# daultanigaurav/AI-BASED-FRAME-INTERPOLATION

Measured on AMD Instinct MI355X. Metric: interpolated frames/sec at 1080p, higher is better.
Workload: dtype bf16

## Files before the change

### ai_based_frame_interpolation_amd/_native.py

```python
from __future__ import annotations

import ctypes
import os
import subprocess

import torch

_PKG = os.path.dirname(os.path.abspath(__file__))
LIB_PATH = os.environ.get("FIUNET_LIB") or os.path.join(_PKG, "libfiunet_hip.so")
CSRC = os.path.join(_PKG, "csrc")

ABI_VERSION = 8
ABI_MIN_COMPAT = 4
FP32, BF16, BF16X2, FP16 = 0, 1, 2, 3
OPT_UNFUSED, OPT_KEEP_ALL, OPT_GATHER_UPSAMPLE = 1, 2, 16
OPT_RNE_WEIGHTS, OPT_NO_DITHER = 32, 64
WEIGHT_PREPS = ("host", "device")
YUV_MPEG2, YUV_BT709, YUV_FULL_RANGE, YUV_BT2020 = 1, 2, 4, 8

SYMBOLS = (
    "fiunet_abi_version", "fiunet_last_error_string", "fiunet_create", "fiunet_destroy",
    "fiunet_set_options", "fiunet_load_weights", "fiunet_load_weights_device", "fiunet_prepare_precision", "fiunet_workspace_bytes", "fiunet_forward",
    "fiunet_min_unsplit_batch",
    "fiunet_forward_strip",
    "fiunet_workspace_bytes_u8", "fiunet_forward_u8", "fiunet_forward_u8_strided", "fiunet_preprocess_u8",
    "fiunet_postprocess_u8", "fiunet_debug_read_activation", "fiunet_profile_enable",
    "fiunet_profile_read", "fiunet_metrics_workspace_bytes", "fiunet_psnr_u8", "fiunet_ssim_u8",
    "fiunet_ssim_gauss_workspace_bytes", "fiunet_ssim_gauss_f32",
    "fiunet_plane_metrics_workspace_bytes", "fiunet_plane_psnr", "fiunet_plane_ssim",
    "fiunet_yuv420_to_rgb_u8", "fiunet_rgb_to_yuv420_u8", "fiunet_workspace_bytes_yuv420", "fiunet_forward_yuv420",
    "fiunet_preprocess_p10", "fiunet_postprocess_p10", "fiunet_workspace_bytes_p10", "fiunet_forward_p10",
    "fiunet_yuv420p10_to_rgb_p10", "fiunet_rgb_p10_to_yuv420p10", "fiunet_workspace_bytes_yuv420p10",
    "fiunet_forward_yuv420p10",
    "fiunet_pair_sad_u8", "fiunet_pair_sad_p10", "fiunet_scene_cuts", "fiunet_hold_cut_frames",
    "fiunet_retime_u8", "fiunet_retime_p10",
    "fiunet_yuv_to_rgb_u8", "fiunet_rgb_to_yuv_u8", "fiunet_yuv_to_rgb_p10", "fiunet_rgb_p10_to_yuv",
    "fiunet_workspace_bytes_yuv", "fiunet_forward_yuv", "fiunet_forward_yuv_p10",
    "fiunet_packed_to_rgb_u8", "fiunet_rgb_to_packed_u8", "fiunet_workspace_bytes_rgb_packed",
    "fiunet_forward_rgb_packed",
    "fiunet_nv12_to_rgb_u8", "fiunet_rgb_to_nv12_u8", "fiunet_workspace_bytes_nv12", "fiunet_forward_nv12",
    "fiunet_p010_to_rgb_p10", "fiunet_rgb_p10_to_p010", "fiunet_workspace_bytes_p010", "fiunet_forward_p010",
)


class SurfaceLayout(ctypes.Structure):
    _fields_ = [("luma_pitch", ctypes.c_size_t), ("chroma_offset", ctypes.c_size_t),
                ("chroma_pitch", ctypes.c_size_t), ("frame_stride", ctypes.c_size_t)]


def _surface(layout, frame_stride: int):
    if layout is None:
        return ctypes.byref(SurfaceLayout(0, 0, 0, frame_stride))
    return ctypes.byref(SurfaceLayout(layout.luma_pitch, layout.chroma_offset, layout.chroma_pitch, frame_stride))



class PackedLayout(ctypes.Structure):
    _fields_ = [("row_pitch", ctypes.c_size_t), ("frame_stride", ctypes.c_size_t)]


def _packed(layout, frame_stride: int):
    return ctypes.byref(PackedLayout(layout.row_pitch, frame_stride))

_lib = None


def build(force: bool = False) -> str:
    if force and os.path.exists(LIB_PATH):
        os.remove(LIB_PATH)
# ... 486 lines not shown
```

### ai_based_frame_interpolation_amd/csrc/conv3x3_mfma.hip.h

```cpp
#pragma once
#include <hip/hip_runtime.h>
#include <stdint.h>
#include <type_traits>

namespace fiunet {

typedef __attribute__((ext_vector_type(4))) float f32x4;
typedef __attribute__((ext_vector_type(8))) __bf16 bf16x8;
typedef __attribute__((ext_vector_type(8))) _Float16 f16x8;

enum SrcMode { SRC_DIRECT = 0, SRC_POOL = 1 , SRC_CONCAT_UP = 2,
               SRC_STEM = 3 ,
               SRC_DIRECT_X2 = 4,
               SRC_STEM_X2 = 5 };
constexpr bool src_is_stem(int mode) { return mode == SRC_STEM || mode == SRC_STEM_X2; }
constexpr bool src_is_x2(int mode) { return mode == SRC_DIRECT_X2 || mode == SRC_STEM_X2; }

__device__ __forceinline__ size_t blk_off(int plane, int y, int x, int H, int W)
{
    return (((size_t)plane * H + y) * W + x) * 64;
}

struct ConvArgs {
    const void* src0;
    const void* src1;
    const void* wgt;
    const float* scale;
    const float* shift;
    void* dst;
    void* pool_dst;
    int B, H, W;
    int C0, C1, Cout;
    int lowH, lowW;
    int padT, padL;
    float sy, sx;
    int upOffY;
    int lowOffY;
    int lowHg;
    int tilesX, tilesY, nct;
    int relu;
    const float* f1;
    const float* f2;
    const void* stem_w;
    float dither;
    int ksplit;
    float* kslab;
    unsigned long long* stamp;
    unsigned stamp_cap;
    const float* head_w;
    const float* head_b;
    float* head_out;
    const uint8_t* u1;
    const uint8_t* u2;
    uint8_t* head_out_u8;
    int head_nc;
    size_t head_img_stride;
};

template <typename T> struct Elem;
template <> struct Elem<float> {
    static constexpr int PL = 16;
    static constexpr int NE = 4;
};
template <> struct Elem<__bf16> {
    static constexpr int PL = 32;
    static constexpr int NE = 8;
};
template <> struct Elem<_Float16> {
    static constexpr int PL = 32;
    static constexpr int NE = 8;
};

template <typename T> __device__ __forceinline__ void chunk_unpack(const uint4& c, float* f);
template <> __device__ __forceinline__ void chunk_unpack<float>(const uint4& c, float* f)
{
    f[0] = __uint_as_float(c.x); f[1] = __uint_as_float(c.y);
    f[2] = __uint_as_float(c.z); f[3] = __uint_as_float(c.w);
}
template <> __device__ __forceinline__ void chunk_unpack<__bf16>(const uint4& c, float* f)
{
    f[0] = __uint_as_float(c.x << 16); f[1] = __uint_as_float(c.x & 0xffff0000u);
    f[2] = __uint_as_float(c.y << 16); f[3] = __uint_as_float(c.y & 0xffff0000u);
    f[4] = __uint_as_float(c.z << 16); f[5] = __uint_as_float(c.z & 0xffff0000u);
    f[6] = __uint_as_float(c.w << 16); f[7] = __uint_as_float(c.w & 0xffff0000u);
}
template <> __device__ __forceinline__ void chunk_unpack<_Float16>(const uint4& c, float* f)
{
    typedef __attribute__((ext_vector_type(2))) _Float16 f16x2;
    const f16x2 a = __builtin_bit_cast(f16x2, c.x), b = __builtin_bit_cast(f16x2, c.y);
    const f16x2 d = __builtin_bit_cast(f16x2, c.z), e = __builtin_bit_cast(f16x2, c.w);
    f[0] = (float)a[0]; f[1] = (float)a[1]; f[2] = (float)b[0]; f[3] = (float)b[1];
    f[4] = (float)d[0]; f[5] = (float)d[1]; f[6] = (float)e[0]; f[7] = (float)e[1];
}
// ... 309 lines not shown
    static constexpr int LDS_BYTES = STEMW_OFF + STEMW_BYTES;
    static_assert(LDS_BYTES <= 80 * 1024, "two workgroups must fit in the CU's 160 KiB of LDS");
    static_assert(!src_is_stem(MODE) || LDS_BYTES <= 63 * 1280, "fused-stem kernel: stay below 64 LDS granules");
};

constexpr int conv_wave_frags(int BN, int TH, int TW) { return TH * TW / 16 / (4 / (BN / 64)); }
constexpr int conv_occupancy(int BN, int TH, int TW, int lds_bytes = 0)
{
    return conv_wave_frags(BN, TH, TW) == 4 && lds_bytes * 3 <= 160 * 1024 ? 3 : 2;
}


__device__ __forceinline__ int conv_block_remap()
{
    const int nblk = gridDim.x, bid = blockIdx.x;
    const int q = nblk >> 3, r = nblk & 7, xcd = bid & 7;
    return (xcd < r ? xcd * (q + 1) : r * (q + 1) + (xcd - r) * q) + (bid >> 3);
}

struct ConvTileId { int ct, b, ty, tx; };
__device__ __forceinline__ ConvTileId conv_tile_decode(const ConvArgs& a, int t)
{
    ConvTileId d;
    d.ct = t % a.nct; t /= a.nct;
    d.tx = t % a.tilesX; t /= a.tilesX;
    d.ty = t % a.tilesY;
    d.b = t / a.tilesY;
    return d;
}

template <typename T> __device__ __forceinline__ int conv_cout_ofs(int m, int lc)
{
    return sizeof(T) == 2 ? (m >> 1) * 32 + lc * 8 + (m & 1) * 4 : m * 16 + lc * 4;
}

template <typename T, int BN, int TH, int TW, int EPI>
__device__ __forceinline__ void conv_acc_init(const ConvArgs& a, f32x4 (&acc)[4][conv_wave_frags(BN, TH, TW)],
                                              int ct, int wc, int lc)
{
    constexpr int NF = conv_wave_frags(BN, TH, TW);
#pragma unroll
    for (int m = 0; m < 4; ++m) {
        f32x4 v = f32x4{0.f, 0.f, 0.f, 0.f};
        if constexpr (!epi_is_splitk(EPI)) {
            const float4 sh = *reinterpret_cast<const float4*>(a.shift + ct * BN + wc * 64 + conv_cout_ofs<T>(m, lc));
            v = f32x4{sh.x, sh.y, sh.z, sh.w};
        }
#pragma unroll
        for (int n = 0; n < NF; ++n) acc[m][n] = v;
    }
}

__device__ __forceinline__ unsigned relu_pk_bf16(unsigned p) { return pk_max_i16(p, 0u); }
__device__ __forceinline__ void relu_fma(float& sum, float x, float lo, float w)
{
    float t;
    asm("v_max_f32 %1, %3, %2\n\tv_fmac_f32 %0, %1, %4" : "+v"(sum), "=&v"(t) : "v"(x), "v"(lo), "v"(w));
}

template <typename T, int BN, int TH, int TW, int EPI, bool X2 = false>
__device__ __forceinline__ void conv_epilogue(const ConvArgs& a, f32x4 (&acc)[4][conv_wave_frags(BN, TH, TW)],
                                              int b, int y0, int x0, int ct, int split, int wc, int wp,
                                              int l15, int lc)
{
    constexpr int PL = Elem<T>::PL;
    constexpr int FR = TW / 16;
    constexpr int NF = conv_wave_frags(BN, TH, TW);
    constexpr int ROWS_W = NF / FR;
    constexpr int HNC = EPI == EPI_HEAD ? 1 : (EPI == EPI_HEAD3 ? 3 : 0);
    const int aH = a.H, aW = a.W;
    constexpr bool PERM = sizeof(T) == 2;
    const int wbase_c = ct * BN + wc * 64;
    if constexpr (epi_is_splitk(EPI)) {
        const int tile = (((b * a.tilesY) + y0 / TH) * a.tilesX + x0 / TW) * a.nct + ct;
        const int ntile = a.B * a.tilesY * a.tilesX * a.nct;
        const int wave = wp * (BN / 64) + wc;
        float4* o = reinterpret_cast<float4*>(a.kslab) + ((((size_t)split * ntile + tile) * 4 + wave) * (4 * NF)) * 64 + (lc * 16 + l15);
#pragma unroll
        for (int m = 0; m < 4; ++m)
#pragma unroll
            for (int n = 0; n < NF; ++n)
                o[(m * NF + n) * 64] = make_float4(acc[m][n][0], acc[m][n][1], acc[m][n][2], acc[m][n][3]);
        return;
    }
    float hw[HNC > 0 ? HNC : 1][4][4];
#pragma unroll
    for (int c = 0; c < HNC; ++c)
#pragma unroll
        for (int m = 0; m < 4; ++m) {
            const float4 v = *reinterpret_cast<const float4*>(a.head_w + c * 64 + conv_cout_ofs<T>(m, lc));
            hw[c][m][0] = v.x; hw[c][m][1] = v.y; hw[c][m][2] = v.z; hw[c][m][3] = v.w;
        }
    const size_t plane_stride = (size_t)aH * aW * 64;
    const int plane0 = wbase_c / PL;
    const int rec_byte = lc * 16;
    char* const out_img = a.dst ? (char*)a.dst + (size_t)b * plane_stride * (a.Cout / PL) +
                                  (size_t)plane0 * plane_stride + rec_byte : nullptr;
    const int pH = aH >> 1, pW = aW >> 1;
    const size_t pplane_stride = (size_t)pH * pW * 64;
    char* const pool_img = EPI == EPI_POOL ? (char*)a.pool_dst + (size_t)b * pplane_stride * (a.Cout / PL) +
                                             (size_t)plane0 * pplane_stride + rec_byte : nullptr;
    if constexpr (HNC > 0) {
        static_assert(HNC == 0 || NF == 8 || NF == 4, "head reduction is written for 8 or 4 fragments per wave");
        const float floor_v = a.relu ? 0.f : -__builtin_inff();
        float hb[HNC];
#pragma unroll
        for (int c = 0; c < HNC; ++c) hb[c] = a.head_b[c];
        const int nb = ((lc & 1) ? 4 : 0) + ((lc & 2) ? 2 : 0);
#pragma unroll
        for (int c = 0; c < HNC; ++c) {
            float hs[NF];
#pragma unroll
            for (int n = 0; n < NF; ++n) {
                float sum = 0.f;
#pragma unroll
                for (int m = 0; m < 4; ++m)
#pragma unroll
                    for (int j = 0; j < 4; ++j) relu_fma(sum, acc[m][n][j], floor_v, hw[c][m][j]);
                hs[n] = sum;
            }
            if constexpr (NF == 4) {
                float full[NF];
#pragma unroll
                for (int n = 0; n < NF; ++n) {
                    const float p = hs[n] + __shfl_xor(hs[n], 16);
                    full[n] = p + __shfl_xor(p, 32);
                }
                const float mine = lc == 0 ? full[0] : (lc == 1 ? full[1] : (lc == 2 ? full[2] : full[3]));
                const int n = lc;
                const int y = y0 + wp * ROWS_W + n / FR;
                const int x = x0 + (n % FR) * 16 + l15;
                if (y < aH && x < aW) {
                    const size_t o = (size_t)b * a.head_img_stride + ((size_t)c * aH + y) * aW + x;
                    if (a.head_out_u8) a.head_out_u8[o] = postprocess_u8_value(mine + hb[c]);
                    else a.head_out[o] = mine + hb[c];
                }
            } else {
                float t[4], u[2];
#pragma unroll
                for (int i = 0; i < 4; ++i) {
                    const auto r = __builtin_amdgcn_permlane16_swap(__float_as_uint(hs[i]), __float_as_uint(hs[(i + 4) % NF]), false, false);
                    t[i] = __uint_as_float(r[0]) + __uint_as_float(r[1]);
                }
#pragma unroll
                for (int j = 0; j < 2; ++j) {
                    const auto r = __builtin_amdgcn_permlane32_swap(__float_as_uint(t[j]), __float_as_uint(t[j + 2]), false, false);
                    u[j] = __uint_as_float(r[0]) + __uint_as_float(r[1]);
                }
#pragma unroll
                for (int j = 0; j < 2; ++j) {
                    const int n = nb + j;
                    const int y = y0 + wp * ROWS_W + n / FR;
                    const int x = x0 + (n % FR) * 16 + l15;
                    if (y < aH && x < aW) {
                        const size_t o = (size_t)b * a.head_img_stride + ((size_t)c * aH + y) * aW + x;
                        if (a.head_out_u8) a.head_out_u8[o] = postprocess_u8_value(u[j] + hb[c]);
                        else a.head_out[o] = u[j] + hb[c];
                    }
                }
            }
        }
    }
    if constexpr (X2) {
        static_assert(std::is_same_v<T, __bf16>, "the two-piece epilogue belongs to the bf16 kernels");
        if (HNC > 0 && !a.dst) return;
        const size_t ps = (size_t)aH * aW * 64;
        const int npo = a.Cout / 32;
        const size_t blk = (size_t)npo * ps;
        char* const img = (char*)a.dst + (size_t)b * 2 * blk + (size_t)(wbase_c / 32) * ps + lc * 16;
        const int pH2 = aH >> 1, pW2 = aW >> 1;
        const size_t pps = (size_t)pH2 * pW2 * 64, pblk = (size_t)npo * pps;
        char* const pimg = EPI == EPI_POOL ? (char*)a.pool_dst + (size_t)b * 2 * pblk + (size_t)(wbase_c / 32) * pps + lc * 16
                                           : nullptr;
        auto put = [&](char* o, size_t block_bytes, const float (&v)[8]) __attribute__((always_inline)) {
            unsigned h[4], l[4];
#pragma unroll
            for (int i = 0; i < 4; ++i) {
                h[i] = pack_bf16x2_pk(v[2 * i], v[2 * i + 1]);
                l[i] = pack_bf16x2_pk(v[2 * i] - __uint_as_float(h[i] << 16), v[2 * i + 1] - __uint_as_float(h[i] & 0xffff0000u));
            }
            *reinterpret_cast<uint4*>(o) = make_uint4(h[0], h[1], h[2], h[3]);
            *reinterpret_cast<uint4*>(o + block_bytes) = make_uint4(l[0], l[1], l[2], l[3]);
        };
#pragma unroll
        for (int n = 0; n < NF; ++n) {
            const int y = y0 + wp * ROWS_W + n / FR;
            const int x = x0 + (n % FR) * 16 + l15;
            if (y < aH && x < aW) {
#pragma unroll
                for (int g = 0; g < 2; ++g) {
                    float v[8];
#pragma unroll
                    for (int j = 0; j < 4; ++j) {
                        v[j] = a.relu ? fmaxf(acc[2 * g][n][j], 0.f) : acc[2 * g][n][j];
                        v[4 + j] = a.relu ? fmaxf(acc[2 * g + 1][n][j], 0.f) : acc[2 * g + 1][n][j];
                    }
                    put(img + (size_t)(y * aW + x) * 64 + g * ps, blk, v);
                }
            }
        }
        if constexpr (EPI == EPI_POOL) {
#pragma unroll
            for (int n = 0; n < NF; ++n) {
                if (((n / FR) & 1) != 0) continue;
                const int y = y0 + wp * ROWS_W + n / FR;
                const int x = x0 + (n % FR) * 16 + l15;
                const int py = y >> 1, px = x >> 1;
                const bool okp = (py < pH2) && (px < pW2) && ((l15 & 1) == 0);
#pragma unroll
                for (int g = 0; g < 2; ++g) {
                    float v[8];
#pragma unroll
                    for (int h = 0; h < 2; ++h)
// ... 10 lines not shown
        }
        return;
    }
    if constexpr (EPI == EPI_POOL && PERM) {
#pragma unroll
        for (int n = 0; n < NF; ++n) {
            if (((n / FR) & 1) != 0) continue;
            uint4 pk[2][2];
#pragma unroll
            for (int r = 0; r < 2; ++r) {
                const int nn = n + r * FR;
                const int y = y0 + wp * ROWS_W + nn / FR;
                const int x = x0 + (nn % FR) * 16 + l15;
                const bool ok = (y < aH) && (x < aW);
                char* o = out_img + (size_t)(y * aW + x) * 64;
#pragma unroll
                for (int g = 0; g < 2; ++g) {
                    uint4 v = make_uint4(pack2_pk<T>(acc[2 * g][nn][0], acc[2 * g][nn][1]),
                                         pack2_pk<T>(acc[2 * g][nn][2], acc[2 * g][nn][3]),
                                         pack2_pk<T>(acc[2 * g + 1][nn][0], acc[2 * g + 1][nn][1]),
                                         pack2_pk<T>(acc[2 * g + 1][nn][2], acc[2 * g + 1][nn][3]));
                    if (a.relu) v = make_uint4(relu_pk_bf16(v.x), relu_pk_bf16(v.y), relu_pk_bf16(v.z), relu_pk_bf16(v.w));
                    pk[r][g] = v;
                    if (ok && out_img) *reinterpret_cast<uint4*>(o + g * plane_stride) = v;
                }
            }
            const int y = y0 + wp * ROWS_W + n / FR;
            const int x = x0 + (n % FR) * 16 + l15;
            const int py = y >> 1, px = x >> 1;
            const bool okp = (py < pH) && (px < pW) && ((l15 & 1) == 0);
            char* o = pool_img + (size_t)(min(py, pH - 1) * pW + min(px, pW - 1)) * 64;
#pragma unroll
            for (int g = 0; g < 2; ++g) {
                const uint4 t = pk[0][g], u = pk[1][g];
                const unsigned c0 = pk_max_i16(t.x, u.x), c1 = pk_max_i16(t.y, u.y);
                const unsigned c2 = pk_max_i16(t.z, u.z), c3 = pk_max_i16(t.w, u.w);
                const uint4 m = make_uint4(pk_max_i16(c0, dpp_swap_pairs(c0)), pk_max_i16(c1, dpp_swap_pairs(c1)),
                                           pk_max_i16(c2, dpp_swap_pairs(c2)), pk_max_i16(c3, dpp_swap_pairs(c3)));
                if (okp) *reinterpret_cast<uint4*>(o + g * pplane_stride) = m;
            }
        }
        return;
    }
#pragma unroll
    for (int n = 0; n < NF; ++n) {
        const int y = y0 + wp * ROWS_W + n / FR;
        const int x = x0 + (n % FR) * 16 + l15;
        const bool ok = (y < aH) && (x < aW);
        if (ok && out_img) {
            char* o = out_img + (size_t)(y * aW + x) * 64;
            if constexpr (PERM) {
#pragma unroll
                for (int g = 0; g < 2; ++g) {
                    uint4 pk = make_uint4(pack2<T>(acc[2 * g][n][0], acc[2 * g][n][1]),
                                          pack2<T>(acc[2 * g][n][2], acc[2 * g][n][3]),
                                          pack2<T>(acc[2 * g + 1][n][0], acc[2 * g + 1][n][1]),
                                          pack2<T>(acc[2 * g + 1][n][2], acc[2 * g + 1][n][3]));
                    if (a.relu) pk = make_uint4(relu_pk_bf16(pk.x), relu_pk_bf16(pk.y), relu_pk_bf16(pk.z), relu_pk_bf16(pk.w));
                    *reinterpret_cast<uint4*>(o + g * plane_stride) = pk;
                }
            } else {
#pragma unroll
                for (int m = 0; m < 4; ++m) {
                    float4 v = make_float4(acc[m][n][0], acc[m][n][1], acc[m][n][2], acc[m][n][3]);
                    if (a.relu) v = make_float4(fmaxf(v.x, 0.f), fmaxf(v.y, 0.f), fmaxf(v.z, 0.f), fmaxf(v.w, 0.f));
                    *reinterpret_cast<float4*>(o + m * plane_stride) = v;
                }
            }
        }
    }
    if (EPI == EPI_POOL) {
#pragma unroll
        for (int n = 0; n < NF; ++n) {
            if (((n / FR) & 1) != 0) continue;
            const int y = y0 + wp * ROWS_W + n / FR;
            const int x = x0 + (n % FR) * 16 + l15;
            const int py = y >> 1, px = x >> 1;
            const bool okp = (py < pH) && (px < pW) && ((l15 & 1) == 0);
            char* o = pool_img + (size_t)(min(py, pH - 1) * pW + min(px, pW - 1)) * 64;
            if constexpr (!PERM) {
#pragma unroll
                for (int m = 0; m < 4; ++m) {
                    float r[4];
#pragma unroll
                    for (int j = 0; j < 4; ++j) {
                        const float cm = fmaxf(acc[m][n][j], acc[m][n + FR][j]);
                        r[j] = fmaxf(cm, __uint_as_float(dpp_swap_pairs(__float_as_uint(cm))));
                        if (a.relu) r[j] = fmaxf(r[j], 0.f);
                    }
                    if (okp) *reinterpret_cast<float4*>(o + m * pplane_stride) = make_float4(r[0], r[1], r[2], r[3]);
                }
            } else {
#pragma unroll
                for (int g = 0; g < 2; ++g) {
                    unsigned r[4];
#pragma unroll
                    for (int h = 0; h < 2; ++h) {
                        const int m = 2 * g + h;
                        const unsigned a0 = pk_max_i16(pack2_pk<T>(acc[m][n][0], acc[m][n][1]),
                                                       pack2_pk<T>(acc[m][n + FR][0], acc[m][n + FR][1]));
                        const unsigned a1 = pk_max_i16(pack2_pk<T>(acc[m][n][2], acc[m][n][3]),
                                                       pack2_pk<T>(acc[m][n + FR][2], acc[m][n + FR][3]));
                        r[2 * h] = pk_max_i16(a0, dpp_swap_pairs(a0));
                        r[2 * h + 1] = pk_max_i16(a1, dpp_swap_pairs(a1));
                        if (a.relu) { r[2 * h] = relu_pk_bf16(r[2 * h]); r[2 * h + 1] = relu_pk_bf16(r[2 * h + 1]); }
                    }
                    if (okp) *reinterpret_cast<uint4*>(o + g * pplane_stride) = make_uint4(r[0], r[1], r[2], r[3]);
                }
            }
        }
// ... 545 lines not shown
                }
            } else {
#pragma unroll
                for (int ky = 0; ky < 3; ++ky) {
                    asm volatile("" ::: "memory");
                    uint4 wa[4], xb[NF];
#pragma unroll
                    for (int m = 0; m < 4; ++m)
                        wa[m] = *reinterpret_cast<const uint4*>(wcur + (ky * BN + m * 16) * 64);
#pragma unroll
                    for (int n = 0; n < NF; ++n)
                        xb[n] = *reinterpret_cast<const uint4*>(
                            lds_in + b_off[kx] + (((n / FR) + ky) * TWP + (n % FR) * 16) * 64);
#pragma unroll
                    for (int m = 0; m < 4; ++m)
#pragma unroll
                        for (int n = 0; n < NF; ++n) mma_chunk<T>(acc[m][n], wa[m], xb[n]);
                }
            }
#ifdef FIUNET_STAMP
            asm volatile("" :: "v"(acc[3][NF - 1][3]));
            __builtin_amdgcn_sched_barrier(0);
#endif
            STAMP(2);
            if (kx == 2 && gather_next && !early) {
                __syncthreads();
                gather_plane(plane + 1, step & 1, false);
                lds_dma_wait_all();
                __syncthreads();
                if constexpr (STEM && X2) { if (plane + 1 == 2) stem_park(1); }
                STAMP(4);
            } else {
                lds_dma_wait_all();
                __syncthreads();
                STAMP(3);
            }
        }
    }

#ifdef FIUNET_CLOCK
    {
        asm volatile("" :: "v"(acc[3][NF - 1][3]));
        __builtin_amdgcn_sched_barrier(0);
        const unsigned long long ck_t1 = __builtin_amdgcn_s_memtime(), ck_r1 = __builtin_amdgcn_s_memrealtime();
        const unsigned st_idx = blockIdx.x * 4u + (unsigned)wave;
        if (a.stamp && lane == 0 && st_idx < a.stamp_cap) {
            unsigned long long* rec = a.stamp + (size_t)st_idx * 16;
            rec[0] = ck_t1 - ck_t0;
            rec[1] = ck_r1 - ck_r0;
            rec[8] = 1ull;
        }
    }
#endif
    conv_epilogue<T, BN, TH, TW, EPI, X2>(a, acc, b, y0, x0, ct, split, wc, wp, l15, lc);
#ifdef FIUNET_STAMP
    STAMP(5);
    st_sum[0] = st_prev - st_t0;
    const unsigned st_idx = blockIdx.x * 4u + (unsigned)wave;
    if (a.stamp && lane == 0 && st_idx < a.stamp_cap) {
        unsigned long long* rec = a.stamp + (size_t)st_idx * 16;
#pragma unroll
        for (int k = 0; k < 16; ++k) rec[k] = k == 8 ? 1ull : st_sum[k];
    }
#endif
}

template <typename T, int BN, int TH, int TW, int EPI, bool X2>
__global__ __launch_bounds__(64) void splitk_finalize_tile_kernel(const ConvArgs a)
{
    static_assert(EPI == EPI_PLAIN || EPI == EPI_POOL, "a fused head is never K-split");
    constexpr int WAVES_C = BN / 64;
    constexpr int NF = conv_wave_frags(BN, TH, TW);
    int t = blockIdx.x >> 2;
    const int tile = t;
    const int ct = t % a.nct; t /= a.nct;
    const int tx = t % a.tilesX; t /= a.tilesX;
    const int ty = t % a.tilesY;
    const int b = t / a.tilesY;
    const int lane = threadIdx.x & 63, wave = blockIdx.x & 3;
    const int l15 = lane & 15, lc = lane >> 4;
    const int wc = wave % WAVES_C, wp = wave / WAVES_C;
    const int ntile = a.B * a.tilesY * a.tilesX * a.nct;
    f32x4 acc[4][NF];
#pragma unroll
    for (int m = 0; m < 4; ++m)
#pragma unroll
        for (int n = 0; n < NF; ++n) acc[m][n] = f32x4{0.f, 0.f, 0.f, 0.f};
    const float4* p = reinterpret_cast<const float4*>(a.kslab) + (((size_t)tile * 4 + wave) * (4 * NF)) * 64 + lane;
    const size_t slice = (size_t)ntile * 4 * (4 * NF) * 64;
    const int ks = a.ksplit;
#pragma unroll
    for (int m = 0; m < 4; ++m) {
        const float4* pm = p + (size_t)m * NF * 64;
        constexpr int CH = NF == 8 ? 2 : 4;
        for (int s0 = 0; s0 < ks; s0 += CH, pm += CH * slice) {
            float4 q[CH][NF];
#pragma unroll
            for (int j = 0; j < CH; ++j)
                if (s0 + j < ks) {
#pragma unroll
                    for (int n = 0; n < NF; ++n) q[j][n] = pm[j * slice + n * 64];
                }
#pragma unroll
            for (int j = 0; j < CH; ++j)
                if (s0 + j < ks) {
#pragma unroll
                    for (int n = 0; n < NF; ++n) {
// ... 18 lines not shown
```

### ai_based_frame_interpolation_amd/csrc/fiunet.hip

```cpp
#include "../../include/fiunet.h"
#include "pointwise.hip.h"
#include "conv3x3_kwave.hip.h"
#include "metrics.hip.h"
#include "colour.hip.h"
#include "packed.hip.h"
#include "yuv4xx.hip.h"
#include "scene.hip.h"
#include "retime.hip.h"
#include "weights.hip.h"

#include <algorithm>
#include <atomic>
#include <cmath>
#include <cstdio>
#include <cstring>
#include <map>
#include <string>
#include <vector>

using namespace fiunet;

namespace {

thread_local std::string g_err;
// ... 539 lines not shown
        HIP_TRY(hipEventRecord(ev[0], s));
    }
    const float dither = bf16 && !(ctx->flags & FIUNET_OPT_NO_DITHER) ? 0.00390625f : 0.f;
    const ConvWeights& c0 = ctx->conv[0];
    const double stem_flops = 2.0 * B * H * W * 9.0 * c0.cin * c0.cout;
    if (L[0].form == STEM_RGB_SPLIT) {
        const long long ntiles = (long long)B * ((H + 15) / 16) * ((W + 31) / 32);
        const dim3 g2((unsigned)std::min<long long>(ntiles, 256 * FIUNET_RGB_STEM_OCC));
        if (x2)
            hipLaunchKernelGGL(stem_rgb_split_kernel<true>, g2, dim3(256), 0, s, f1, f2, (const float*)c0.w_f32, c0.scale,
                               c0.shift, (__bf16*)act(0), B, H, W, dither, u1, u2);
        else if (f16)
            hipLaunchKernelGGL((stem_rgb_split_kernel<false, _Float16>), g2, dim3(256), 0, s, f1, f2, (const float*)c0.w_f32, c0.scale,
                               c0.shift, (_Float16*)act(0), B, H, W, 0.f, u1, u2);
        else
            hipLaunchKernelGGL(stem_rgb_split_kernel<false>, g2, dim3(256), 0, s, f1, f2, (const float*)c0.w_f32, c0.scale,
                               c0.shift, (__bf16*)act(0), B, H, W, dither, u1, u2);
        HIP_TRY(hipGetLastError());
    } else if (L[0].form == STEM_FIRST) {
        const long long nruns = (long long)B * H * (((W + 15) / 16 + 7) / 8);
        const dim3 grid((unsigned)std::min<long long>((nruns + 3) / 4, 256 * 64));
        if (x2)
            hipLaunchKernelGGL((conv3x3_first_kernel<__bf16, 1, true>), grid, dim3(256), 0, s, f1, f2, (const float*)c0.w_f32,
                               c0.scale, c0.shift, (__bf16*)act(0), B, H, W, dither);
        else if (ctx->cf == 1)
            hipLaunchKernelGGL((conv3x3_first_kernel<T, 1>), grid, dim3(256), 0, s, f1, f2, (const float*)c0.w_f32, c0.scale,
                               c0.shift, (T*)act(0), B, H, W, dither);
        else if constexpr (sizeof(T) == 4)
            hipLaunchKernelGGL((conv3x3_first_kernel<T, 3>), grid, dim3(256), 0, s, f1, f2, (const float*)c0.w_f32, c0.scale,
                               c0.shift, (T*)act(0), B, H, W, dither);
        HIP_TRY(hipGetLastError());
    }
    if (ev) {
        HIP_TRY(hipEventRecord(ev[1], s));
        if (L[0].form == STEM_FUSED) ctx->layer_name[0] = "(stem fused into next stage)";
        else if (x2) ctx->layer_name[0] = L[0].form == STEM_FIRST ? "conv3x3_first_kernel<f32 arithmetic, two-piece output>"
                                                                  : "stem_rgb_split_kernel<two-piece output>";
        else ctx->layer_name[0] = L[0].form == STEM_FIRST ? std::string("conv3x3_first_kernel<") + elem_name<T>() + "," +
                                                                std::to_string(ctx->cf) + ">"
                                                          : std::string(f16 ? "stem_rgb_split_kernel<fp16 output>" : "stem_rgb_split_kernel");
        ctx->layer_flops[0] = L[0].form == STEM_FUSED ? 0.0 : stem_flops;
    }
    for (int i = 1; i < NCONV; ++i) {
        const StageLaunch& st = L[i];
        const ConvWeights& cw = ctx->conv[i];
        const int lv = kLevel[i];
        ConvArgs a;
        std::memset(&a, 0, sizeof(a));
        a.B = B; a.H = p.hs[lv]; a.W = p.ws[lv];
        a.Cout = cw.cout;
        a.wgt = x2 ? cw.w_x2 : bf16 ? cw.w_bf16 : f16 ? cw.w_f16 : cw.w_f32;
        a.scale = cw.scale; a.shift = cw.shift;
        a.relu = 1;
        a.ksplit = 1;
        a.kslab = st.slab ? (float*)(ws + p.slab_off) : nullptr;
        a.stamp = (ctx->stamps && i == ctx->stamp_layer) ? ctx->stamps : nullptr;
        a.stamp_cap = (unsigned)kStampWaves;
        a.dst = st.stored ? act(i) : nullptr;
        a.src0 = act(kSrc0[i]);
        a.C0 = ctx->cout[kSrc0[i]];
        int mode = x2 ? SRC_DIRECT_X2 : SRC_DIRECT;
        if (st.form == FORM_POOL) {
            char* pooled = ws + p.pool_off[lv - 1];
            if (L[i - 1].epi != EPI_POOL) {
                const size_t n = (size_t)B * a.H * a.W * (a.C0 * sizeof(T) / 16);
                hipLaunchKernelGGL((maxpool2_kernel<T>), dim3(grid_for(n)), dim3(256), 0, s,
                                   (const T*)a.src0, (T*)pooled, B, p.hs[lv - 1], p.ws[lv - 1], a.C0);
                HIP_TRY(hipGetLastError());
            }
            a.src0 = pooled;
        } else if (kMode[i] == SRC_CONCAT_UP) {
            a.src1 = act(kSrc1[i]);
            a.C1 = ctx->cout[kSrc1[i]];
            a.lowH = p.hs[lv + 1]; a.lowW = p.ws[lv + 1];
            a.lowHg = hg[lv + 1];
            a.upOffY = y_origin >> lv;
            a.lowOffY = y_origin >> (lv + 1);
            const int dy = hg[lv] - 2 * a.lowHg, dx = a.W - 2 * a.lowW;
            a.padT = dy / 2; a.padL = dx / 2;
            a.sy = 2 * a.lowHg > 1 ? (float)(a.lowHg - 1) / (float)(2 * a.lowHg - 1) : 0.f;
            a.sx = 2 * a.lowW > 1 ? (float)(a.lowW - 1) / (float)(2 * a.lowW - 1) : 0.f;
            char* up = ws + p.up_off[i];
            if (st.form == FORM_CONCAT_CONVT) {
                const auto& ct = ctx->convt[(i - 10) / 2];
                ConvTArgs c;
                std::memset(&c, 0, sizeof(c));
                c.low = a.src1; c.wgt = x2 ? ct.w_x2 : bf16 ? ct.w_bf16 : f16 ? ct.w_f16 : ct.w_f32; c.bias = ct.bias; c.dst = up;
                c.B = B; c.H = a.H; c.W = a.W; c.lowH = a.lowH; c.lowW = a.lowW; c.Cin = ct.cin; c.Cout = ct.cout;
                c.padT = a.padT; c.padL = a.padL; c.upOffY = a.upOffY; c.lowOffY = a.lowOffY; c.lowHg = a.lowHg;
                if (a.C1 != ct.cin) return fail(FIUNET_ERR_INVALID_ARG, "internal: transposed-conv channel plan mismatch");
                if (y_origin != 0 || Hg != H || a.H != 2 * a.lowH || a.W != 2 * a.lowW)
                    HIP_TRY(hipMemsetAsync(up, 0, (size_t)B * a.H * a.W * ct.cout * es, s));
                const long long units = (long long)B * a.lowH * ((a.lowW + 31) / 32) * (ct.cout / 64);
                const dim3 grid((unsigned)std::min<long long>((units + 3) / 4, 256 * 16));
                if (x2) {
                    if constexpr (std::is_same_v<T, __bf16>) hipLaunchKernelGGL((convt2x2_kernel<T, true>), grid, dim3(256), 0, s, c);
                } else
                    hipLaunchKernelGGL((convt2x2_kernel<T>), grid, dim3(256), 0, s, c);
                HIP_TRY(hipGetLastError());
                a.src1 = up; a.C1 = ct.cout;
            } else if (st.form == FORM_CONCAT_UPCAT) {
                T* scratch = (T*)(ws + p.scratch_off);
                const size_t n = (size_t)B * a.H * a.W * ((a.C0 + a.C1) * sizeof(T) / 16);
                hipLaunchKernelGGL((upcat_kernel<T>), dim3(grid_for(n)), dim3(256), 0, s, a, scratch);
                HIP_TRY(hipGetLastError());
                a.src0 = scratch; a.C0 = a.C0 + a.C1; a.C1 = 0; a.src1 = nullptr;
// ... 1531 lines not shown
    return retime(grid, n_intervals, frame_samples, depth, first_interval, j0, n_out, p, q, mode, flags, out, stream);
}

int fiunet_retime_p10(const uint16_t* grid, int n_intervals, size_t frame_samples, int depth, uint64_t first_interval,
                      uint64_t j0, int n_out, uint32_t p, uint32_t q, int mode, const uint8_t* flags, uint16_t* out,
                      void* stream)
{
    return retime(grid, n_intervals, frame_samples, depth, first_interval, j0, n_out, p, q, mode, flags, out, stream);
}

int fiunet_debug_force_cfg(fiunet_ctx* ctx, int layer, int tile, int ksplit)
{
    if (!ctx || layer >= NCONV || tile < 0 || tile > 3 || ksplit < 0 || ksplit > 32)
        return fail(FIUNET_ERR_INVALID_ARG, "fiunet_debug_force_cfg: bad arguments");
    if (layer < 0) {
        for (int i = 0; i < NCONV; ++i) ctx->force_tile[i] = ctx->force_ksplit[i] = 0;
        return FIUNET_OK;
    }
    ctx->force_tile[layer] = tile;
    ctx->force_ksplit[layer] = ksplit;
    return FIUNET_OK;
}

int fiunet_debug_weight_buffer(const fiunet_ctx* ctx, int layer, int which, const void** ptr, size_t* bytes)
{
    if (!ctx || !ptr || !bytes || layer < 0 || layer > NCONV + 4 || which < 0 || which > 5)
        return fail(FIUNET_ERR_INVALID_ARG, "fiunet_debug_weight_buffer: bad arguments");
    if (!ctx->loaded) return fail(FIUNET_ERR_NOT_LOADED, "fiunet_debug_weight_buffer before a load");
    const void* p = nullptr;
    size_t b = 0;
    if (layer < NCONV) {
        const ConvWeights& cw = ctx->conv[layer];
        const size_t nel = (size_t)9 * cw.cin * cw.cout;
        if (which == 0) { p = cw.scale; b = (size_t)cw.cout * 4; }
        else if (which == 1) { p = cw.shift; b = (size_t)cw.cout * 4; }
        else if (which == 2) { p = cw.w_f32; b = nel * 4; }
        else if (which == 3) { p = cw.w_bf16; b = nel * 2; }
        else if (which == 4 && layer == 0) { p = ctx->stem_w_split; b = (size_t)2 * 64 * 32 * 2; }
    } else if (layer < NCONV + 4) {
        const auto& ct = ctx->convt[layer - NCONV];
        const size_t nel = (size_t)4 * ct.cin * ct.cout;
        if (which == 2) { p = ct.w_f32; b = nel * 4; }
        else if (which == 3) { p = ct.w_bf16; b = nel * 2; }
        else if (which == 5) { p = ct.bias; b = (size_t)ct.cout * 4; }
    } else {
        if (which == 2) { p = ctx->head_w; b = (size_t)ctx->cf * 64 * 4; }
        else if (which == 5) { p = ctx->head_b; b = (size_t)ctx->cf * 4; }
    }
    *ptr = p;
    *bytes = p ? b : 0;
    return FIUNET_OK;
}

int fiunet_debug_choose_cfg(int precision, int B, int H, int W, int Cin, int Cout, int splittable, int concat_stage,
                            int kwave_ok, int* out )
{
    if (!out || B < 1 || H < 1 || W < 1 || Cin < 32 || (Cout != 64 && Cout % 128 != 0) || !valid_precision(precision))
        return fail(FIUNET_ERR_INVALID_ARG, "fiunet_debug_choose_cfg: bad arguments");
    const bool concat = concat_stage >= 10;
    out[3] = concat && concat_stage < NCONV && kMode[concat_stage] == SRC_CONCAT_UP &&
             (precision == FIUNET_BF16X2 ||
              materialise_up(precision, B, H, W, conv_cin(kCoutBil, true, concat_stage), kCoutBil[concat_stage]));
    const ConvCfg c = choose_conv_cfg(precision == FIUNET_FP32, precision == FIUNET_BF16X2, B, H, W, Cin, Cout, splittable != 0,
                                      -1, 0, concat ? out[3] != 0 : kwave_ok != 0, kwave_ok != 0,
                                      concat && !(precision == FIUNET_FP32 && out[3]));
    out[0] = c.small; out[1] = c.ksplit; out[2] = c.kwave;
    return FIUNET_OK;
}

int fiunet_debug_stage_cfg(int frame_channels, int bilinear, unsigned flags, int precision, int B, int H, int W, int stage,
                           int* out )
{
    if (!out || (frame_channels != 1 && frame_channels != 3) || B < 1 || H < 16 || W < 16 || stage < 0 || stage >= NCONV ||
        !valid_precision(precision))
        return fail(FIUNET_ERR_INVALID_ARG, "fiunet_debug_stage_cfg: bad arguments");
    NetDesc n;
    n.cf = frame_channels;
    n.bilinear = bilinear != 0;
    n.cout = n.bilinear ? kCoutBil : kCoutCT;
    n.flags = flags;
    n.stem_w = frame_channels == 1;
    StageLaunch L[NCONV];
    plan_stages(n, precision, B, H, W, L);
    const StageLaunch& st = L[stage];
    out[0] = st.cfg.small; out[1] = st.cfg.ksplit; out[2] = st.cfg.kwave;
    out[3] = stage > 0 && (st.form == FORM_CONCAT_UP || st.form == FORM_CONCAT_CONVT);
    out[4] = st.form; out[5] = st.epi;
    return FIUNET_OK;
}

int fiunet_debug_plan(int frame_channels, int bilinear, unsigned flags, int precision, int B, int H, int W,
                      long long* records , int capacity, int* n_records, unsigned long long* total)
{
    if (!records || capacity < 0 || !n_records || !total || (frame_channels != 1 && frame_channels != 3) || B < 1 || H < 16 ||
        W < 16 || !valid_precision(precision))
        return fail(FIUNET_ERR_INVALID_ARG, "fiunet_debug_plan: bad arguments");
    NetDesc n;
    n.cf = frame_channels;
    n.bilinear = bilinear != 0;
    n.cout = n.bilinear ? kCoutBil : kCoutCT;
    n.flags = flags;
    n.stem_w = frame_channels == 1;
    Plan p;
    std::vector<PlanBuf> bufs;
    if (!make_plan(n, B, H, W, precision, p, &bufs)) return fail(FIUNET_ERR_BAD_SHAPE, "fiunet_debug_plan: bad shape");
    *n_records = (int)bufs.size();
// ... 126 lines not shown
```

### ai_based_frame_interpolation_amd/unet.py

```python
from __future__ import annotations

import os

import torch
import torch.nn as nn

from . import _native

_ENCODER = (("down1", 64, 128), ("down2", 128, 256), ("down3", 256, 512), ("down4", 512, 512))
_DECODER = (("up1", 1024, 256), ("up2", 512, 128), ("up3", 256, 64), ("up4", 128, 64))
_ENCODER_CT = (("down1", 64, 128), ("down2", 128, 256), ("down3", 256, 512), ("down4", 512, 1024))
_DECODER_CT = (("up1", 1024, 512), ("up2", 512, 256), ("up3", 256, 128), ("up4", 128, 64))

TAP_CHANNELS = (64, 64, 128, 128, 256, 256, 512, 512, 512, 512, 512, 256, 256, 128, 128, 64, 64, 64)
TAP_CHANNELS_CT = (64, 64, 128, 128, 256, 256, 512, 512, 1024, 1024, 512, 512, 256, 256, 128, 128, 64, 64)
TAP_LEVEL = (0, 0, 1, 1, 2, 2, 3, 3, 4, 4, 3, 3, 2, 2, 1, 1, 0, 0)
TAP_NAMES = tuple(
    f"{p}.double_conv.{c}"
    for p in ("unet.inc", "unet.down1.maxpool_conv.1", "unet.down2.maxpool_conv.1",
              "unet.down3.maxpool_conv.1", "unet.down4.maxpool_conv.1", "unet.up1.conv",
              "unet.up2.conv", "unet.up3.conv", "unet.up4.conv")
    for c in (0, 3))

UP_TAP_NAMES = ("unet.up1.up", "unet.up2.up", "unet.up3.up", "unet.up4.up")
# ... 89 lines not shown
        self.frame_channels = frame_channels
        self.precision = precision or os.environ.get("FIUNET_PRECISION", "fp32")
        if self.precision not in _PRECISIONS:
            raise ValueError(f"precision must be one of {sorted(_PRECISIONS)}")
        self.weight_prep = weight_prep or os.environ.get("FIUNET_WEIGHT_PREP", "host")
        self._weight_prep_checked()
        self._prep_loaded = None
        self._ctx = None
        self._ctx_dirty = True
        self._weights_gen = 0
        self._tracked = None
        self._fingerprint = None
        self._ws = None
        self._options = 0

    def _apply(self, fn, *a, **k):
        self._ctx_dirty = True
        self._tracked = None
        return super()._apply(fn, *a, **k)

    def _current_fingerprint(self):
        tracked = list(self.parameters()) + list(self.buffers())
        fp = []
        for t in tracked:
            try:
                ver = t._version
            except RuntimeError:
                ver = 0
            fp.append((id(t), ver, t.data_ptr()))
        return tuple(fp)

    def __getstate__(self):
        st = self.__dict__.copy()
        st["_ctx"], st["_ws"], st["_tracked"], st["_fingerprint"], st["_ctx_dirty"] = None, None, None, None, True
        return st

    def __deepcopy__(self, memo):
        import copy
        new = self.__class__.__new__(self.__class__)
        memo[id(self)] = new
        for k, v in self.__getstate__().items():
            new.__dict__[k] = copy.deepcopy(v, memo)
        return new

    def load_state_dict(self, *a, **k):
        self._ctx_dirty = True
        self._tracked = None
        return super().load_state_dict(*a, **k)

    def refresh_weights(self):
        self._ctx_dirty = True

    def set_options(self, *, unfused: bool = False, keep_all: bool = False, gather_upsample: bool = False,
                    rne_weights: bool = False, no_dither: bool = False):
        old = self._options
        self._options = ((_native.OPT_UNFUSED if unfused else 0) | (_native.OPT_KEEP_ALL if keep_all else 0)
                         | (_native.OPT_GATHER_UPSAMPLE if gather_upsample else 0)
                         | (_native.OPT_RNE_WEIGHTS if rne_weights else 0)
                         | (_native.OPT_NO_DITHER if no_dither else 0))
        if (old ^ self._options) & _native.OPT_RNE_WEIGHTS:
            self._ctx_dirty = True
        if self._ctx is not None:
            self._ctx.set_options(self._options)

    def _ctx_or_none_set_options(self):
        if self._ctx is not None:
            self._ctx.set_options(self._options)

    def _context(self, device: torch.device) -> "_native.Context":
        idx = device.index if device.index is not None else torch.cuda.current_device()
        if self._ctx is None or self._ctx.device_index != idx:
            if self._ctx is not None:
                self._ctx.close()
            self._ctx = _native.Context(idx, self.frame_channels, self.unet.bilinear)
            self._ctx_dirty = True
        fp = self._current_fingerprint()
        prep = self._weight_prep_checked()
        if self._ctx_dirty or fp != self._fingerprint or prep != self._prep_loaded:
            self._ctx.set_options(self._options)
            self._ctx.load_state_dict(self.state_dict(), prep=prep)
            self._ctx_dirty = False
            self._prep_loaded = prep
            self._fingerprint = fp
            self._weights_gen += 1
        return self._ctx

    def _workspace(self, ctx, device, b, h, w, prec, u8=False, yuv=False, p10=False):
        nbytes = ctx.workspace_bytes(b, h, w, prec, u8, yuv, p10)
        if self._ws is None or self._ws.device != device or self._ws.numel() < nbytes:
            self._ws = None
            self._ws = torch.empty(nbytes, dtype=torch.uint8, device=device)
        return self._ws

    def _weight_prep_checked(self) -> str:
        if self.weight_prep not in _native.WEIGHT_PREPS:
            raise ValueError(f"weight_prep must be one of {list(_native.WEIGHT_PREPS)}, got {self.weight_prep!r}")
        return self.weight_prep

    def _precision_code(self) -> int:
        try:
            return _PRECISIONS[self.precision]
        except (KeyError, TypeError):
            raise ValueError(f"precision must be one of {sorted(_PRECISIONS)}, got {self.precision!r}") from None

    def _check_pair(self, frame1, frame2, dtype_ok):
        if frame1.dim() != 4 or frame1.shape != frame2.shape:
            raise RuntimeError(
                f"expected two [B,{self.frame_channels},H,W] tensors of equal shape, got "
                f"{tuple(frame1.shape)} and {tuple(frame2.shape)}")
        if frame1.shape[1] != self.frame_channels:
            raise RuntimeError(
                f"expected {self.frame_channels} channel(s) per frame, got {frame1.shape[1]}")
# ... 275 lines not shown
```

### include/fiunet.h

```cpp
#ifndef FIUNET_H
#define FIUNET_H

#include <stddef.h>
#include <stdint.h>

#ifdef __cplusplus
extern "C" {
#endif

#define FIUNET_ABI_VERSION 8

enum fiunet_status {
    FIUNET_OK = 0,
    FIUNET_ERR_INVALID_ARG = 1,
    FIUNET_ERR_BAD_SHAPE = 2,
    FIUNET_ERR_MISSING_WEIGHT = 3,
    FIUNET_ERR_NOT_LOADED = 4,
    FIUNET_ERR_WORKSPACE = 5,
    FIUNET_ERR_HIP = 6,
    FIUNET_ERR_UNSUPPORTED = 7
};

enum fiunet_precision {
    FIUNET_FP32 = 0,
    FIUNET_BF16 = 1,
    FIUNET_BF16X2 = 2,
    FIUNET_FP16 = 3
};

enum fiunet_option {
    FIUNET_OPT_UNFUSED = 1,
    FIUNET_OPT_KEEP_ALL = 2,
    FIUNET_OPT_RNE_WEIGHTS = 32,
    FIUNET_OPT_NO_DITHER = 64,
    FIUNET_OPT_GATHER_UPSAMPLE = 16
};

typedef struct fiunet_ctx fiunet_ctx;

int fiunet_create(fiunet_ctx** out_ctx, int device_id, int frame_channels, int bilinear);

int fiunet_destroy(fiunet_ctx* ctx);

int fiunet_set_options(fiunet_ctx* ctx, unsigned flags);

int fiunet_load_weights(fiunet_ctx* ctx, int n, const char* const* names,
                        const float* const* host_ptrs, const int64_t* numels);

int fiunet_load_weights_device(fiunet_ctx* ctx, int n, const char* const* names,
                               const float* const* device_ptrs, const int64_t* numels, void* stream);

int fiunet_prepare_precision(fiunet_ctx* ctx, int precision);

size_t fiunet_workspace_bytes(const fiunet_ctx* ctx, int B, int H, int W, int precision);

int fiunet_min_unsplit_batch(const fiunet_ctx* ctx, int H, int W, int precision);

int fiunet_forward(fiunet_ctx* ctx, const float* frame1, const float* frame2, float* out, int B,
                   int H, int W, int precision, void* workspace, size_t workspace_bytes,
                   void* stream);

int fiunet_forward_strip(fiunet_ctx* ctx, const float* frame1, const float* frame2, float* out, int B,
                         int H, int W, int y_origin, int H_image, int precision, void* workspace,
                         size_t workspace_bytes, void* stream);

size_t fiunet_workspace_bytes_u8(const fiunet_ctx* ctx, int B, int H, int W, int precision);
int fiunet_forward_u8(fiunet_ctx* ctx, const uint8_t* frame1, const uint8_t* frame2, uint8_t* out,
                      int B, int H, int W, int precision, void* workspace, size_t workspace_bytes,
                      void* stream);
int fiunet_forward_u8_strided(fiunet_ctx* ctx, const uint8_t* frame1, const uint8_t* frame2, uint8_t* out,
                              size_t out_image_stride, int B, int H, int W, int precision, void* workspace,
                              size_t workspace_bytes, void* stream);

enum fiunet_colour {
    FIUNET_YUV_MPEG2 = 1,
    FIUNET_YUV_BT709 = 2,
    FIUNET_YUV_FULL_RANGE = 4,
    FIUNET_YUV_BT2020 = 8
};

int fiunet_yuv420_to_rgb_u8(const uint8_t* in, size_t in_frame_stride, uint8_t* out, int B, int H, int W,
                            unsigned colour, void* stream);
int fiunet_rgb_to_yuv420_u8(const uint8_t* in, uint8_t* out, size_t out_frame_stride, int B, int H, int W,
                            unsigned colour, void* stream);
size_t fiunet_workspace_bytes_yuv420(const fiunet_ctx* ctx, int B, int H, int W, int precision);
int fiunet_forward_yuv420(fiunet_ctx* ctx, const uint8_t* frame1, const uint8_t* frame2, uint8_t* out,
                          size_t out_frame_stride, int B, int H, int W, unsigned colour, int precision,
                          void* workspace, size_t workspace_bytes, void* stream);
// ... 136 lines not shown
```

Baseline: 529.9.

## Add bounds-free interior-tile fast path to conv epilogue stores and pooling

Adds an interior-tile path to the conv epilogue. When a wave's output rows lie fully inside the image (and are pool-aligned when pooling), it writes packed bf16/fp16 records with precomputed lane offsets, fuses the 2x2 max-pool through DPP swaps, and skips per-element bounds checks. The head reduction now does all four ReLU-FMAs for a fragment in one inline asm block, and non-head layers use the packed conversion. This is meant to cut address arithmetic and branching in the store phase, at the cost of a second code path that can diverge from the boundary path and raises code size and register pressure. A new option flag can turn the path off.

```diff
diff --git a/ai_based_frame_interpolation_amd/_native.py b/ai_based_frame_interpolation_amd/_native.py
--- a/ai_based_frame_interpolation_amd/_native.py
+++ b/ai_based_frame_interpolation_amd/_native.py
@@ -15,6 +15,7 @@
 FP32, BF16, BF16X2, FP16 = 0, 1, 2, 3
 OPT_UNFUSED, OPT_KEEP_ALL, OPT_GATHER_UPSAMPLE = 1, 2, 16
 OPT_RNE_WEIGHTS, OPT_NO_DITHER = 32, 64
+OPT_NO_INTERIOR_PATH = 128
 WEIGHT_PREPS = ("host", "device")
 YUV_MPEG2, YUV_BT709, YUV_FULL_RANGE, YUV_BT2020 = 1, 2, 4, 8
 
diff --git a/ai_based_frame_interpolation_amd/csrc/conv3x3_mfma.hip.h b/ai_based_frame_interpolation_amd/csrc/conv3x3_mfma.hip.h
--- a/ai_based_frame_interpolation_amd/csrc/conv3x3_mfma.hip.h
+++ b/ai_based_frame_interpolation_amd/csrc/conv3x3_mfma.hip.h
@@ -39,6 +39,7 @@
     int lowHg;
     int tilesX, tilesY, nct;
     int relu;
+    int interior;
     const float* f1;
     const float* f2;
     const void* stem_w;
@@ -454,13 +455,43 @@
 }
 
 __device__ __forceinline__ unsigned relu_pk_bf16(unsigned p) { return pk_max_i16(p, 0u); }
-__device__ __forceinline__ void relu_fma(float& sum, float x, float lo, float w)
+__device__ __forceinline__ void relu_fma4(float& sum, const f32x4& x, float lo, const float (&w)[4])
 {
     float t;
-    asm("v_max_f32 %1, %3, %2\n\tv_fmac_f32 %0, %1, %4" : "+v"(sum), "=&v"(t) : "v"(x), "v"(lo), "v"(w));
-}
-
-template <typename T, int BN, int TH, int TW, int EPI, bool X2 = false>
+    asm("v_max_f32 %1, %6, %2\n\tv_fmac_f32 %0, %1, %7\n\t"
+        "v_max_f32 %1, %6, %3\n\tv_fmac_f32 %0, %1, %8\n\t"
+        "v_max_f32 %1, %6, %4\n\tv_fmac_f32 %0, %1, %9\n\t"
+        "v_max_f32 %1, %6, %5\n\tv_fmac_f32 %0, %1, %10"
+        : "+v"(sum), "=&v"(t)
+        : "v"(x[0]), "v"(x[1]), "v"(x[2]), "v"(x[3]), "v"(lo), "v"(w[0]), "v"(w[1]), "v"(w[2]), "v"(w[3]));
+}
+
+__device__ __forceinline__ unsigned fresh_lane_id()
+{
+    unsigned l;
+    asm volatile("v_mbcnt_lo_u32_b32 %0, -1, 0\n\tv_mbcnt_hi_u32_b32 %0, -1, %0" : "=v"(l));
+    return l;
+}
+
+__host__ __device__ constexpr bool tile_store_interior(int y0, int x0, int th, int tw, int H, int W, bool pool)
+{
+    return y0 >= 0 && x0 >= 0 && y0 + th <= H && x0 + tw <= W &&
+           (!pool || ((y0 & 1) == 0 && (x0 & 1) == 0 && (y0 + th + 1) / 2 <= H / 2 && (x0 + tw + 1) / 2 <= W / 2));
+}
+
+template <typename T, bool PK> __device__ __forceinline__ unsigned pack2x(float lo, float hi)
+{
+    if constexpr (PK) return pack2_pk<T>(lo, hi);
+    else return pack2<T>(lo, hi);
+}
+template <typename T, bool PK>
+__device__ __forceinline__ uint4 pack_record(const f32x4& lo, const f32x4& hi, unsigned fl)
+{
+    return make_uint4(pk_max_i16(pack2x<T, PK>(lo[0], lo[1]), fl), pk_max_i16(pack2x<T, PK>(lo[2], lo[3]), fl),
+                      pk_max_i16(pack2x<T, PK>(hi[0], hi[1]), fl), pk_max_i16(pack2x<T, PK>(hi[2], hi[3]), fl));
+}
+
+template <typename T, int BN, int TH, int TW, int EPI, bool X2 = false, bool INTERIOR = true>
 __device__ __forceinline__ void conv_epilogue(const ConvArgs& a, f32x4 (&acc)[4][conv_wave_frags(BN, TH, TW)],
                                               int b, int y0, int x0, int ct, int split, int wc, int wp,
                                               int l15, int lc)
@@ -485,6 +516,8 @@
                 o[(m * NF + n) * 64] = make_float4(acc[m][n][0], acc[m][n][1], acc[m][n][2], acc[m][n][3]);
         return;
     }
+    const int yw = y0 + wp * ROWS_W;
+    const bool interior = INTERIOR && PERM && !X2 && a.interior && tile_store_interior(yw, x0, ROWS_W, TW, aH, aW, EPI == EPI_POOL);
     float hw[HNC > 0 ? HNC : 1][4][4];
 #pragma unroll
     for (int c = 0; c < HNC; ++c)
@@ -516,9 +549,7 @@
             for (int n = 0; n < NF; ++n) {
                 float sum = 0.f;
 #pragma unroll
-                for (int m = 0; m < 4; ++m)
-#pragma unroll
-                    for (int j = 0; j < 4; ++j) relu_fma(sum, acc[m][n][j], floor_v, hw[c][m][j]);
+                for (int m = 0; m < 4; ++m) relu_fma4(sum, acc[m][n], floor_v, hw[c][m]);
                 hs[n] = sum;
             }
             if constexpr (NF == 4) {
@@ -532,7 +563,12 @@
                 const int n = lc;
                 const int y = y0 + wp * ROWS_W + n / FR;
                 const int x = x0 + (n % FR) * 16 + l15;
-                if (y < aH && x < aW) {
+                if (interior) {
+                    const size_t o = (size_t)b * a.head_img_stride + ((size_t)c * aH + yw) * aW + x0;
+                    const unsigned lo = (unsigned)((n / FR) * aW + (n % FR) * 16 + l15);
+                    if (a.head_out_u8) (a.head_out_u8 + o)[lo] = postprocess_u8_value(mine + hb[c]);
+                    else (a.head_out + o)[lo] = mine + hb[c];
+                } else if (y < aH && x < aW) {
                     const size_t o = (size_t)b * a.head_img_stride + ((size_t)c * aH + y) * aW + x;
                     if (a.head_out_u8) a.head_out_u8[o] = postprocess_u8_value(mine + hb[c]);
                     else a.head_out[o] = mine + hb[c];
@@ -549,6 +585,16 @@
                     const auto r = __builtin_amdgcn_permlane32_swap(__float_as_uint(t[j]), __float_as_uint(t[j + 2]), false, false);
                     u[j] = __uint_as_float(r[0]) + __uint_as_float(r[1]);
                 }
+                if (interior) {
+                    const size_t o = (size_t)b * a.head_img_stride + ((size_t)c * aH + yw) * aW + x0;
+#pragma unroll
+                    for (int j = 0; j < 2; ++j) {
+                        const int n = nb + j;
+                        const unsigned lo = (unsigned)((n / FR) * aW + (n % FR) * 16 + l15);
+                        if (a.head_out_u8) (a.head_out_u8 + o)[lo] = postprocess_u8_value(u[j] + hb[c]);
+                        else (a.head_out + o)[lo] = u[j] + hb[c];
+                    }
+                } else
 #pragma unroll
                 for (int j = 0; j < 2; ++j) {
                     const int n = nb + j;
@@ -561,6 +607,56 @@
                     }
                 }
             }
+        }
+    }
+    if constexpr (INTERIOR && PERM && !X2) {
+        if (interior) {
+            const unsigned fl = a.relu ? 0u : 0x80008000u;
+            const unsigned ln = fresh_lane_id();
+            const unsigned loff = (ln & 15u) * 64u + (ln >> 4) * 16u;
+            const unsigned row_bytes = (unsigned)aW * 64u;
+            char* const ob = a.dst ? (char*)a.dst + ((size_t)b * (a.Cout / PL) + plane0) * plane_stride +
+                                     ((size_t)yw * aW + x0) * 64 : nullptr;
+            if constexpr (EPI == EPI_POOL) {
+                const unsigned prow_bytes = (unsigned)pW * 64u;
+                const unsigned ploff = ((ln & 15u) >> 1) * 64u + (ln >> 4) * 16u;
+                char* const pb = (char*)a.pool_dst + ((size_t)b * (a.Cout / PL) + plane0) * pplane_stride +
+                                 ((size_t)(yw >> 1) * pW + (x0 >> 1)) * 64;
+                char* const obg[2] = {ob, ob ? ob + plane_stride : nullptr};
+                char* const pbg[2] = {pb, pb + pplane_stride};
+#pragma unroll
+                for (int n = 0; n < NF; ++n) {
+                    if (((n / FR) & 1) != 0) continue;
+                    uint4 m[2];
+#pragma unroll
+                    for (int g = 0; g < 2; ++g) {
+                        const uint4 t = pack_record<T, true>(acc[2 * g][n], acc[2 * g + 1][n], fl);
+                        const uint4 u = pack_record<T, true>(acc[2 * g][n + FR], acc[2 * g + 1][n + FR], fl);
+                        if (ob) {
+                            char* const o = obg[g] + (size_t)(n / FR) * row_bytes + (n % FR) * 1024;
+                            *reinterpret_cast<uint4*>(o + loff) = t;
+                            *reinterpret_cast<uint4*>(o + row_bytes + loff) = u;
+                        }
+                        const unsigned c0 = pk_max_i16(t.x, u.x), c1 = pk_max_i16(t.y, u.y);
+                        const unsigned c2 = pk_max_i16(t.z, u.z), c3 = pk_max_i16(t.w, u.w);
+                        m[g] = make_uint4(pk_max_i16(c0, dpp_swap_pairs(c0)), pk_max_i16(c1, dpp_swap_pairs(c1)),
+                                          pk_max_i16(c2, dpp_swap_pairs(c2)), pk_max_i16(c3, dpp_swap_pairs(c3)));
+                    }
+                    if ((ln & 1u) == 0) {
+                        *reinterpret_cast<uint4*>(pbg[0] + (size_t)(n / FR / 2) * prow_bytes + (n % FR) * 512 + ploff) = m[0];
+                        *reinterpret_cast<uint4*>(pbg[1] + (size_t)(n / FR / 2) * prow_bytes + (n % FR) * 512 + ploff) = m[1];
+                    }
+                }
+            } else if (ob) {
+                char* const obg[2] = {ob, ob + plane_stride};
+#pragma unroll
+                for (int n = 0; n < NF; ++n)
+#pragma unroll
+                    for (int g = 0; g < 2; ++g)
+                        *reinterpret_cast<uint4*>(obg[g] + (size_t)(n / FR) * row_bytes + (n % FR) * 1024 + loff) =
+                            pack_record<T, HNC == 0>(acc[2 * g][n], acc[2 * g + 1][n], fl);
+            }
+            return;
         }
     }
     if constexpr (X2) {
@@ -677,10 +773,11 @@
             if constexpr (PERM) {
 #pragma unroll
                 for (int g = 0; g < 2; ++g) {
-                    uint4 pk = make_uint4(pack2<T>(acc[2 * g][n][0], acc[2 * g][n][1]),
-                                          pack2<T>(acc[2 * g][n][2], acc[2 * g][n][3]),
-                                          pack2<T>(acc[2 * g + 1][n][0], acc[2 * g + 1][n][1]),
-                                          pack2<T>(acc[2 * g + 1][n][2], acc[2 * g + 1][n][3]));
+                    constexpr bool PK = HNC == 0;
+                    uint4 pk = make_uint4(pack2x<T, PK>(acc[2 * g][n][0], acc[2 * g][n][1]),
+                                          pack2x<T, PK>(acc[2 * g][n][2], acc[2 * g][n][3]),
+                                          pack2x<T, PK>(acc[2 * g + 1][n][0], acc[2 * g + 1][n][1]),
+                                          pack2x<T, PK>(acc[2 * g + 1][n][2], acc[2 * g + 1][n][3]));
                     if (a.relu) pk = make_uint4(relu_pk_bf16(pk.x), relu_pk_bf16(pk.y), relu_pk_bf16(pk.z), relu_pk_bf16(pk.w));
                     *reinterpret_cast<uint4*>(o + g * plane_stride) = pk;
                 }
@@ -1332,7 +1429,8 @@
         }
     }
 #endif
-    conv_epilogue<T, BN, TH, TW, EPI, X2>(a, acc, b, y0, x0, ct, split, wc, wp, l15, lc);
+    constexpr bool EPI_INTERIOR = !(STEM && std::is_same_v<T, _Float16>);
+    conv_epilogue<T, BN, TH, TW, EPI, X2, EPI_INTERIOR>(a, acc, b, y0, x0, ct, split, wc, wp, l15, lc);
 #ifdef FIUNET_STAMP
     STAMP(5);
     st_sum[0] = st_prev - st_t0;
diff --git a/ai_based_frame_interpolation_amd/csrc/fiunet.hip b/ai_based_frame_interpolation_amd/csrc/fiunet.hip
--- a/ai_based_frame_interpolation_amd/csrc/fiunet.hip
+++ b/ai_based_frame_interpolation_amd/csrc/fiunet.hip
@@ -615,6 +615,7 @@
         a.wgt = x2 ? cw.w_x2 : bf16 ? cw.w_bf16 : f16 ? cw.w_f16 : cw.w_f32;
         a.scale = cw.scale; a.shift = cw.shift;
         a.relu = 1;
+        a.interior = !(ctx->flags & FIUNET_OPT_NO_INTERIOR_PATH);
         a.ksplit = 1;
         a.kslab = st.slab ? (float*)(ws + p.slab_off) : nullptr;
         a.stamp = (ctx->stamps && i == ctx->stamp_layer) ? ctx->stamps : nullptr;
@@ -2252,6 +2253,20 @@
     return FIUNET_OK;
 }
 
+int fiunet_debug_tile_class(int H, int W, int th, int tw, int rows_w, int pool, unsigned char* out, size_t cap)
+{
+    if (!out || H < 1 || W < 1 || th < 1 || tw < 1 || rows_w < 1 || th % rows_w)
+        return fail(FIUNET_ERR_INVALID_ARG, "fiunet_debug_tile_class: bad arguments");
+    const int tilesX = (W + tw - 1) / tw, tilesY = (H + th - 1) / th, nb = th / rows_w;
+    if ((size_t)tilesX * tilesY * nb > cap) return fail(FIUNET_ERR_INVALID_ARG, "fiunet_debug_tile_class: out too small");
+    for (int ty = 0; ty < tilesY; ++ty)
+        for (int tx = 0; tx < tilesX; ++tx)
+            for (int k = 0; k < nb; ++k)
+                out[((size_t)ty * tilesX + tx) * nb + k] =
+                    tile_store_interior(ty * th + k * rows_w, tx * tw, rows_w, tw, H, W, pool != 0);
+    return FIUNET_OK;
+}
+
 int fiunet_debug_choose_cfg(int precision, int B, int H, int W, int Cin, int Cout, int splittable, int concat_stage,
                             int kwave_ok, int* out )
 {
diff --git a/ai_based_frame_interpolation_amd/unet.py b/ai_based_frame_interpolation_amd/unet.py
--- a/ai_based_frame_interpolation_amd/unet.py
+++ b/ai_based_frame_interpolation_amd/unet.py
@@ -165,12 +165,13 @@
         self._ctx_dirty = True
 
     def set_options(self, *, unfused: bool = False, keep_all: bool = False, gather_upsample: bool = False,
-                    rne_weights: bool = False, no_dither: bool = False):
+                    rne_weights: bool = False, no_dither: bool = False, no_interior_path: bool = False):
         old = self._options
         self._options = ((_native.OPT_UNFUSED if unfused else 0) | (_native.OPT_KEEP_ALL if keep_all else 0)
                          | (_native.OPT_GATHER_UPSAMPLE if gather_upsample else 0)
                          | (_native.OPT_RNE_WEIGHTS if rne_weights else 0)
-                         | (_native.OPT_NO_DITHER if no_dither else 0))
+                         | (_native.OPT_NO_DITHER if no_dither else 0)
+                         | (_native.OPT_NO_INTERIOR_PATH if no_interior_path else 0))
         if (old ^ self._options) & _native.OPT_RNE_WEIGHTS:
             self._ctx_dirty = True
         if self._ctx is not None:
diff --git a/include/fiunet.h b/include/fiunet.h
--- a/include/fiunet.h
+++ b/include/fiunet.h
@@ -33,7 +33,8 @@
     FIUNET_OPT_KEEP_ALL = 2,
     FIUNET_OPT_RNE_WEIGHTS = 32,
     FIUNET_OPT_NO_DITHER = 64,
-    FIUNET_OPT_GATHER_UPSAMPLE = 16
+    FIUNET_OPT_GATHER_UPSAMPLE = 16,
+    FIUNET_OPT_NO_INTERIOR_PATH = 128
 };
 
 typedef struct fiunet_ctx fiunet_ctx;
```

Result: no change. 529.2 (-0.1%).
